# wusize/CLIPSelf

Hardware: AMD Instinct MI355X
Metric: images/sec (student+teacher distill step), ViT-B/16 32 crops/img (higher is better)
Workload: dtype bf16; 1 GPU; EVA02-CLIP-B-16 CLIPSelf image-patches step, 64 images x 32 crops per GPU, 224^2 (BASELINE configs[1]); global_batch=64, crops_per_image=32, image_size=224, parallelism=dp1, teacher_chunk=2048, teacher_last_block=cls_query_only, teacher_schedule=one_batch_ahead_on_side_stream

## Files before the change

### clipself_amd/csrc/gemm_stream.hip

```cpp
#include <vector>
#include <cstdio>
#include "gemm_common.h"

namespace {

typedef __attribute__((ext_vector_type(2))) unsigned u32x2;
typedef __attribute__((ext_vector_type(4))) unsigned u32x4;

constexpr unsigned OOB = 0xfffffff0u;

__device__ __forceinline__ float lane_bcast(int src_lane_x4, float v) {
    return __int_as_float(__builtin_amdgcn_ds_bpermute(src_lane_x4, __float_as_int(v)));
}
__device__ __forceinline__ unsigned pack2(float a, float b) {
    union { bf16x2 v; unsigned u; } pk;
    pk.v[0] = f2bf(a);
    pk.v[1] = f2bf(b);
    return pk.u;
}
__device__ __forceinline__ void swap32(unsigned& x, unsigned& y) {
    const u32x2 r = __builtin_amdgcn_permlane32_swap(x, y, false, false);
    x = r[0];
    y = r[1];
}
// ... 356 lines not shown

template <bool LN, bool AUX, int CP>
__device__ __forceinline__ void epi_swiglu_slab(const GemmArgs& p, const f32x16 (&acc)[4][2], int lane, int row0, int tn, int wn, const EpiOps& eo,
                                                char* slab) {
    const int l31 = lane & 31, hf = lane >> 5;
    const int hbase = tn * 128 + wn * 32;
    const bool colok = hbase < p.group;
    float nm[4], rs[4];
#pragma unroll
    for (int i = 0; i < 4; ++i) {
        rs[i] = LN ? eo.rstd[i] : 1.f;
        nm[i] = LN ? -eo.rstd[i] * eo.mean[i] : 0.f;
    }
    float ssum[4] = {0.f, 0.f, 0.f, 0.f}, ssq[4] = {0.f, 0.f, 0.f, 0.f};
    const int sl0 = hf << 4;
#pragma unroll
    for (int q = 0; q < 4; ++q) {
        float hv[4][4];
#pragma unroll
        for (int r = 0; r < 4; ++r) {
            const int e = q * 4 + r;
            const int sl = sl0 + ((8 * q + r) << 2);
            const float b1 = lane_bcast(sl, eo.cb), b2 = lane_bcast(sl + 128, eo.cb);
            float c1 = 0.f, c2 = 0.f;
            if (LN) { c1 = lane_bcast(sl, eo.cc); c2 = lane_bcast(sl + 128, eo.cc); }
#pragma unroll
            for (int i = 0; i < 4; ++i) {
                float u = acc[i][0][e], v = acc[i][1][e];
                if (LN) {
                    u = fmaf(rs[i], u, fmaf(nm[i], c1, b1));
                    v = fmaf(rs[i], v, fmaf(nm[i], c2, b2));
                } else {
                    u += b1;
                    v += b2;
                }
                hv[i][r] = silu_mul(u, v);
            }
        }
#pragma unroll
        for (int i = 0; i < 4; ++i) {
            const unsigned d0 = pack2(hv[i][0], hv[i][1]), d1 = pack2(hv[i][2], hv[i][3]);
            if (AUX) {
                ssum[i] = dot2_bf16(d1, 0x3f803f80u, dot2_bf16(d0, 0x3f803f80u, ssum[i]));
                ssq[i] = dot2_bf16(d1, d1, dot2_bf16(d0, d0, ssq[i]));
            }
            const int lrow = i * 32 + l31;
            const int s8 = (2 * q + hf) ^ (((lrow >> 1) & 3) << 1);
            *(uint2*)(slab + lrow * 64 + s8 * 8) = make_uint2(d0, d1);
        }
    }
    const __amdgpu_buffer_rsrc_t rc = make_rsrc((const __bf16*)p.C + (size_t)row0 * p.ldc + hbase);
    const int piece = lane & 3;
#pragma unroll
    for (int k = 0; k < 8; ++k) {
        const int lrow = (lane >> 2) + 16 * k;
        const uint4 w = *(const uint4*)(slab + lrow * 64 + ((piece ^ ((lrow >> 1) & 3)) << 4));
        const bool ok = colok && row0 + lrow < p.M && !CS_ABL(p, 8);
        store16<CP>(u32x4{w.x, w.y, w.z, w.w}, rc, ok ? (unsigned)(lrow * p.ldc + piece * 8) * 2u : OOB);
    }
    if (AUX) {
        const size_t slice = (size_t)tn * 4 + wn;
        const __amdgpu_buffer_rsrc_t rst = make_rsrc(p.stats_part + (slice * p.M + row0) * 2);
#pragma unroll
        for (int i = 0; i < 4; ++i) {
            const float s = both_halves(ssum[i]), q2 = both_halves(ssq[i]);
            const bool ok = colok && hf == 0 && row0 + i * 32 + l31 < p.M && !CS_ABL(p, 8);
            store8<CP>(u32x2{__float_as_uint(s), __float_as_uint(q2)}, rst, ok ? (unsigned)(i * 32 + l31) * 8u : OOB);
        }
    }
}

#ifdef CS_ABLATION_SWITCHES
__device__ unsigned long long* g_epi_trace = nullptr;
#define EPI_TRACE(slot)                                                                                                            \
    do {                                                                                                                           \
        if (g_epi_trace && (threadIdx.x & 63) == 0)                                                                                \
            g_epi_trace[((size_t)blockIdx.x * 8 + (threadIdx.x >> 6)) * 16 + (slot)] = __builtin_amdgcn_s_memrealtime();           \
    } while (0)
#define EPI_TRACE_WAIT() do { if (g_epi_trace) asm volatile("s_waitcnt vmcnt(0)" ::: "memory"); } while (0)
#else
#define EPI_TRACE(slot) do { } while (0)
#define EPI_TRACE_WAIT() do { } while (0)
#endif
template <bool LN, bool AUX, int CP, bool F8 = false, int SPLIT = 0, int FM = 4>
__device__ __forceinline__ void epi_resid_slab(const GemmArgs& p, const f32x16 (&acc)[FM][2], int lane, int row0, int colw, int tn, int wn,
                                               const EpiOps& eo, char* slab) {
    static_assert(!(SPLIT & 2) || AUX, "a split stream leaves together with the row statistics");
    const int l31 = lane & 31, hf = lane >> 5;
    const int rrow = lane >> 3, piece = lane & 7, col = colw + piece * 8;
    const bool colok = col < p.N;
    const __amdgpu_buffer_rsrc_t rc = make_rsrc((SPLIT & 2) ? (const void*)p.xb_out : (const void*)((const float*)p.C + (size_t)row0 * p.ldc + colw));
    const __amdgpu_buffer_rsrc_t rx = make_rsrc((SPLIT & 1) ? (const void*)p.xb_out : (const void*)(p.extra + (size_t)row0 * p.ldc + colw));
    const __amdgpu_buffer_rsrc_t rb = make_rsrc((AUX || SPLIT) ? (const void*)(p.xb_out + (size_t)row0 * p.ldxb + colw) : (const void*)p.C);
    const __amdgpu_buffer_rsrc_t rl = make_rsrc(SPLIT ? (const void*)(p.lo + (size_t)row0 * p.ldxb + colw) : (const void*)p.A);
    const size_t slice = (size_t)tn * 4 + wn;
    const __amdgpu_buffer_rsrc_t rst = make_rsrc(AUX ? (const void*)(p.stats_part + (slice * p.M + row0) * 2) : (const void*)p.C);
    f32x4 cb4[2] = {{0.f, 0.f, 0.f, 0.f}, {0.f, 0.f, 0.f, 0.f}}, cc4[2] = {{0.f, 0.f, 0.f, 0.f}, {0.f, 0.f, 0.f, 0.f}};
#pragma unroll
    for (int h = 0; h < 2; ++h) {
        const unsigned off = colok ? (unsigned)(col + 4 * h) * 4u : OOB;
        if (p.bias) cb4[h] = __builtin_bit_cast(f32x4, __builtin_amdgcn_raw_buffer_load_b128(make_rsrc(p.bias), off, 0, 0));
        if (LN || F8) cc4[h] = __builtin_bit_cast(f32x4, __builtin_amdgcn_raw_buffer_load_b128(make_rsrc(p.ln_colsum), off, 0, 0));
    }
    EPI_TRACE(0);
#pragma unroll
    for (int i = 0; i < FM; ++i) {
        f32x4 xin[4][2];
#pragma unroll
        for (int it = 0; it < 4; ++it) {
            const int rrel = i * 32 + rrow + 8 * it;
            const bool ok = colok && row0 + rrel < p.M;
            if constexpr (SPLIT & 1) {
                const unsigned off = ok ? (unsigned)(rrel * p.ldxb + piece * 8) * 2u : OOB;
                const u32x4 h = __builtin_bit_cast(u32x4, __builtin_amdgcn_raw_buffer_load_b128(rb, off, 0, CP));
                const u32x4 l = __builtin_bit_cast(u32x4, __builtin_amdgcn_raw_buffer_load_b128(rl, off, 0, CP));
#pragma unroll
                for (int w = 0; w < 4; ++w) {
                    xin[it][w >> 1][2 * (w & 1)] = __uint_as_float(__builtin_amdgcn_perm(h[w], l[w], 0x05040100u) - 0x8000u);
                    xin[it][w >> 1][2 * (w & 1) + 1] = __uint_as_float(__builtin_amdgcn_perm(h[w], l[w], 0x07060302u) - 0x8000u);
                }
            } else {
                const unsigned off = ok ? (unsigned)(rrel * p.ldc + piece * 8) * 4u : OOB;
                xin[it][0] = __builtin_bit_cast(f32x4, __builtin_amdgcn_raw_buffer_load_b128(rx, off, 0, CP));
                xin[it][1] = __builtin_bit_cast(f32x4, __builtin_amdgcn_raw_buffer_load_b128(rx, ok ? off + 16u : OOB, 0, CP));
            }
        }
        const float rs_row = (LN || F8) ? eo.rstd[i] : 1.f, nm_row = LN ? -eo.rstd[i] * eo.mean[i] : 0.f;
#pragma unroll
        for (int j = 0; j < 2; ++j)
#pragma unroll
            for (int q = 0; q < 4; ++q) {
                f32x4 t;
#pragma unroll
                for (int r = 0; r < 4; ++r) t[r] = acc[i][j][q * 4 + r];
                const int s16 = (j * 8 + 2 * q + hf) ^ (l31 & 15);
                *(f32x4*)(slab + l31 * 256 + s16 * 16) = t;
            }
        EPI_TRACE(1 + 3 * i);
        EPI_TRACE_WAIT();
        EPI_TRACE(2 + 3 * i);
        const int sel = lane & 7;
        float st_s = 0.f, st_q = 0.f;
#pragma unroll
        for (int it = 0; it < 4; ++it) {
            const int lrow = rrow + 8 * it, rrel = i * 32 + lrow;
            const bool ok = colok && row0 + rrel < p.M;
            float rs = 1.f, nm = 0.f;
            if (LN || F8) rs = lane_bcast(lrow << 2, rs_row);
            if (LN) nm = lane_bcast(lrow << 2, nm_row);
            f32x4 o[2];
#pragma unroll
            for (int h = 0; h < 2; ++h) {
                const f32x4 sv = *(const f32x4*)(slab + lrow * 256 + (((2 * piece + h) ^ (lrow & 15)) << 4));
                if (LN) {
#pragma unroll
                    for (int t = 0; t < 4; ++t) o[h][t] = xin[it][h][t] + fmaf(rs, sv[t], fmaf(nm, cc4[h][t], cb4[h][t]));
                } else if (F8) {
#pragma unroll
                    for (int t = 0; t < 4; ++t) o[h][t] = xin[it][h][t] + fmaf(rs * cc4[h][t], sv[t], cb4[h][t]);
                } else {
                    o[h] = xin[it][h] + (sv + cb4[h]);
                }
            }
            if constexpr (SPLIT & 2) {
                const unsigned off = ok ? (unsigned)(rrel * p.ldxb + piece * 8) * 2u : OOB;
                unsigned y[8];
#pragma unroll
                for (int t = 0; t < 8; ++t) y[t] = __float_as_uint(o[t >> 2][t & 3]) + 0x8000u;
                store16<CP>(u32x4{__builtin_amdgcn_perm(y[1], y[0], 0x07060302u), __builtin_amdgcn_perm(y[3], y[2], 0x07060302u),
                                  __builtin_amdgcn_perm(y[5], y[4], 0x07060302u), __builtin_amdgcn_perm(y[7], y[6], 0x07060302u)}, rb, off);
                store16<CP>(u32x4{__builtin_amdgcn_perm(y[1], y[0], 0x05040100u), __builtin_amdgcn_perm(y[3], y[2], 0x05040100u),
                                  __builtin_amdgcn_perm(y[5], y[4], 0x05040100u), __builtin_amdgcn_perm(y[7], y[6], 0x05040100u)}, rl, off);
            } else {
                const unsigned off = ok ? (unsigned)(rrel * p.ldc + piece * 8) * 4u : OOB;
                store16<CP>(__builtin_bit_cast(u32x4, o[0]), rc, off);
                store16<CP>(__builtin_bit_cast(u32x4, o[1]), rc, ok ? off + 16u : OOB);
            }
            if (AUX) {
                if constexpr (!(SPLIT & 2))
                    store16<CP>(u32x4{pack2(o[0][0], o[0][1]), pack2(o[0][2], o[0][3]), pack2(o[1][0], o[1][1]), pack2(o[1][2], o[1][3])}, rb,
                                ok ? (unsigned)(rrel * p.ldxb + piece * 8) * 2u : OOB);
                float ps = 0.f, pq = 0.f;
                if (colok) {
#pragma unroll
                    for (int t = 0; t < 8; ++t) { ps += o[t >> 2][t & 3]; pq = fmaf(o[t >> 2][t & 3], o[t >> 2][t & 3], pq); }
                }
                const float a = sum_lanes8(ps), b = sum_lanes8(pq);
                if (sel == it) { st_s = a; st_q = b; }
            }
        }
        if (AUX) {
            const int rrel = i * 32 + rrow + 8 * sel;
            const bool ok = sel < 4 && row0 + rrel < p.M && colw < p.N;
            store8<CP>(u32x2{__float_as_uint(st_s), __float_as_uint(st_q)}, rst, ok ? (unsigned)rrel * 8u : OOB);
        }
        EPI_TRACE(3 + 3 * i);
        __builtin_amdgcn_sched_barrier(0);
    }
}

template <int EPI, bool AUX, bool SLAB, int SPLIT = 0, int FM = 4, int MF = 32>
constexpr int epi_stores() {
    if (EPI == EPI_SWIGLU_BF16 && MF == 16) return 8 + (AUX ? 2 : 0);
    if (EPI == EPI_SWIGLU_BF16) return FM * (2 + (AUX ? 1 : 0));
    if (EPI == EPI_RESID_F32) return FM * (8 + (AUX ? ((SPLIT & 2) ? 0 : 4) + 1 : 0));
    return FM * 4;
}

#ifndef CS_DMA_AUX_A
#define CS_DMA_AUX_A 0
#endif
#ifndef CS_DMA_AUX_B
#define CS_DMA_AUX_B 0
#endif
#define CS_VMCNT(N) asm volatile("s_waitcnt vmcnt(%0)" ::"n"(N) : "memory")

inline bool getenv_flag(const char* name) {
    const char* v = getenv(name);
    return v && v[0] && v[0] != '0';
}

template <int EPI, bool LN, bool AUX, bool SLAB, bool F8 = false, int SPLIT = 0, int BMT = 256, int MF = 32>
__global__ __launch_bounds__(512) void gemm_stream_kernel(GemmArgs p) {
    static_assert(MF == 32 || (MF == 16 && LN && !SLAB && !F8 && SPLIT == 0 && BMT == 256 && (epi_is_bf16(EPI) ? !AUX : EPI == EPI_SWIGLU_BF16)),
                  "16x16x32 loop: the folded-LN bf16 and SwiGLU register epilogues");
    constexpr bool M16 = MF == 16;
    static_assert(BMT == 256 || (BMT == 192 && !F8 && SPLIT == 0 && !LN && !AUX), "192-row tiles: the training schedule's plain epilogues");
    static_assert(SPLIT == 0 || (EPI == EPI_RESID_F32 && LN && !F8), "the split stream belongs to the folded-LayerNorm residual epilogue");
    static_assert(SLAB || EPI != EPI_RESID_F32, "the fp32 residual epilogue exists in the slab form only (whole-line traffic)");
    static_assert(!F8 || (!LN && !AUX && (EPI == EPI_BF16 || EPI == EPI_RESID_F32)), "fp8 operands: bf16 and fp32-residual outputs");
    constexpr int ES = F8 ? 1 : 2;
    constexpr int CP = 0;
    constexpr bool SWI = EPI == EPI_SWIGLU_BF16, RES = EPI == EPI_RESID_F32;
    static_assert(SWI || RES || epi_is_bf16(EPI), "register epilogues");
    constexpr int BM = BMT, BN = 256, WN = 4, TM = BM / 2, TN = 64, FM = TM / 32, FN = 2;
    constexpr int A_BYTES = BM * BK * 2, B_BYTES = BN * BK * 2;
    constexpr int NPA = BM / 32;
    constexpr int NM = FM * FN, NR = FM + FN;
    constexpr int S = epi_stores<EPI, AUX, SLAB, SPLIT, FM, MF>() < 55 ? epi_stores<EPI, AUX, SLAB, SPLIT, FM, MF>() : 55;
    extern __shared__ __attribute__((aligned(16))) char smem[];
    const int tid = threadIdx.x, lane = tid & 63;
    const int wave = __builtin_amdgcn_readfirstlane(tid >> 6);
    const int wm = wave / WN, wn = wave - wm * WN;
    const int hf = M16 ? lane >> 4 : lane >> 5, l31 = M16 ? lane & 15 : lane & 31;
    char* const b_ring = smem + 3 * A_BYTES;
    const int ntiles = p.tiles_m * p.tiles_n, ktiles = p.K / (F8 ? 128 : BK);
    const int a_base = ((wm * TM + l31) >> 1) << 8, b_base = ((wn * TN + l31) >> 1) << 8;
    const int par8 = (l31 & 1) << 3, sw = l31 >> 1;
    const int G = gridDim.x;
#ifndef CS_NO_DMA_ROLES
    constexpr bool ROLES = !F8;
#else
    constexpr bool ROLES = false;
#endif
    const bool role_a = ROLES && wave >= 4;
#ifndef CS_NO_MID_BARRIER
    constexpr bool MID = ROLES && !SLAB && !F8;
#else
    constexpr bool MID = false;
#endif

    unsigned avoff[ROLES ? 8 : 4], bvoff[ROLES ? 1 : 4];
    const char *a_src = nullptr, *b_src = nullptr;
    int a_tile = blockIdx.x, a_kt = 0, b_tile = blockIdx.x, b_kt = 0;
    auto set_a = [&](int tile) {
        int tm, tn;
        tile_of_id(p, tile, ntiles, tm, tn);
        a_src = (const char*)p.A + (size_t)tm * BM * p.lda * ES;
#pragma unroll
        for (int i = 0; i < (ROLES ? NPA : 4); ++i) {
            int tr, chk;
            lane_source(ROLES ? (wave & 3) * NPA + i : wave * 4 + i, lane, tr, chk);
            avoff[i] = (unsigned)(min(tr, p.M - 1 - tm * BM) * p.lda * ES + chk * 16);
        }
    };
    auto set_b = [&](int tile) {
        int tm, tn;
        tile_of_id(p, tile, ntiles, tm, tn);
        if (SWI) {
            b_src = (const char*)p.B + (size_t)tn * (BN / 2) * p.ldb * ES;
        } else {
            b_src = (const char*)p.B + (size_t)tn * BN * p.ldb * ES;
        }
#pragma unroll
        for (int i = 0; i < (ROLES ? 8 : 4); ++i) {
            int tr, chk;
            lane_source(ROLES ? (wave & 3) * 8 + i : wave * 4 + i, lane, tr, chk);
            int rel;
            if (SWI) {
                const int hrel = (tr >> 6) * 32 + (tr & 31);
                rel = ((tr >> 5) & 1) * p.group + min(hrel, p.group - 1 - tn * (BN / 2));
            } else {
                rel = min(tr, p.N - 1 - tn * BN);
            }
            (ROLES ? avoff : bvoff)[i] = (unsigned)(rel * p.ldb * ES + chk * 16);
        }
    };
    auto adv_a = [&]() {
        if (++a_kt == ktiles) {
            a_kt = 0;
            if (a_tile + G < ntiles) {
                a_tile += G;
                set_a(a_tile);
            }
        }
    };
    auto adv_b = [&]() {
        if (++b_kt == ktiles) {
            b_kt = 0;
            if (b_tile + G < ntiles) {
                b_tile += G;
                set_b(b_tile);
            }
        }
    };
#define ISSUE_A(X, SLOT)                                                                                                      \
    __builtin_amdgcn_global_load_lds((const __attribute__((address_space(1))) void*)(a_src + (size_t)a_kt * (BK * 2) + avoff[X]), \
                                     (__attribute__((address_space(3))) void*)(smem + (SLOT) * A_BYTES + (wave * 4 + (X)) * 1024), 16, 0, CS_DMA_AUX_A)
#define ISSUE_B(X, SLOT)                                                                                                      \
    __builtin_amdgcn_global_load_lds((const __attribute__((address_space(1))) void*)(b_src + (size_t)b_kt * (BK * 2) + bvoff[X]), \
                                     (__attribute__((address_space(3))) void*)(b_ring + (SLOT) * B_BYTES + (wave * 4 + (X)) * 1024), 16, 0, CS_DMA_AUX_B)

#define ISSUE_RA(X, SLOT)                                                                                                     \
    __builtin_amdgcn_global_load_lds((const __attribute__((address_space(1))) void*)(a_src + (size_t)a_kt * (BK * 2) + avoff[X]), \
                                     (__attribute__((address_space(3))) void*)(smem + (SLOT) * A_BYTES + ((wave & 3) * NPA + (X)) * 1024), 16, 0, CS_DMA_AUX_A)
#define ISSUE_RB(X, SLOT)                                                                                                     \
    __builtin_amdgcn_global_load_lds((const __attribute__((address_space(1))) void*)(b_src + (size_t)b_kt * (BK * 2) + avoff[X]), \
                                     (__attribute__((address_space(3))) void*)(b_ring + (SLOT) * B_BYTES + ((wave & 3) * 8 + (X)) * 1024), 16, 0, CS_DMA_AUX_B)

    if constexpr (ROLES) {
        if (role_a) {
            set_a(a_tile);
#pragma unroll
            for (int x = 0; x < NPA; ++x) ISSUE_RA(x, 0);
            adv_a();
#pragma unroll
            for (int x = 0; x < NPA; ++x) ISSUE_RA(x, 1);
            adv_a();
        } else {
            set_b(b_tile);
#pragma unroll
            for (int x = 0; x < 8; ++x) ISSUE_RB(x, 0);
            adv_b();
            if constexpr (MID) {
#pragma unroll
                for (int x = 0; x < 8; ++x) ISSUE_RB(x, 1);
                adv_b();
            }
        }
        if constexpr (MID) {
            if (role_a) CS_VMCNT(NPA);
            else CS_VMCNT(8);
            __builtin_amdgcn_s_barrier();
        }
    } else {
        set_a(a_tile);
        set_b(b_tile);
#pragma unroll
        for (int x = 0; x < 4; ++x) ISSUE_A(x, 0);
        adv_a();
#pragma unroll
        for (int x = 0; x < 4; ++x) ISSUE_B(x, 0);
        adv_b();
#pragma unroll
        for (int x = 0; x < 4; ++x) ISSUE_A(x, 1);
        adv_a();
    }

    int curA = 0, gpar = 0;
    bool after_epi = false;
    for (int tile = blockIdx.x; tile < ntiles; tile += G) {
        int tm, tn;
        tile_of_id(p, tile, ntiles, tm, tn);
        const int row0 = tm * BM + wm * TM, colw = tn * BN + wn * TN;
        f32x16 acc[M16 ? 1 : FM][M16 ? 1 : FN];
        f32x4 acc16[M16 ? 8 : 1][M16 ? 4 : 1];
        constexpr int RB = M16 ? 16 : 32, NRB = TM / RB;
        EpiOpsT<M16 ? 8 : 4> eo;
        auto load_epi_ops = [&](int ln) {
            const int l31 = ln & (RB - 1), hf = ln >> 5, lane = ln;
#pragma unroll
            for (int i = 0; i < (M16 ? 8 : 4); ++i) eo.mean[i] = eo.rstd[i] = 0.f;
            eo.cb = eo.cc = 0.f;
            if (LN || F8) {
#pragma unroll
                for (int i = 0; i < NRB; ++i) {
                    const int r = min(row0 + i * RB + l31, p.M - 1);
                    if (LN) eo.mean[i] = p.ln_mean[r];
                    eo.rstd[i] = p.ln_rstd[r];
                }
            }
            int co;
            if (SWI) co = hf * p.group + min(tn * 128 + wn * 32 + (lane & 31), p.group - 1);
            else co = min(colw + lane, p.N - 1);
            if (!RES) {
                if (p.bias) eo.cb = p.bias[co];
                if (LN || F8) eo.cc = p.ln_colsum[co];
            }
        };

        auto ktile = [&](auto zero_tag, auto role_tag) {
            constexpr bool ZERO = decltype(zero_tag)::value;
            constexpr int ROLE = decltype(role_tag)::value;
            constexpr int KEEP = ROLE == 0 ? 4 : ROLE == 1 ? 0 : NPA;
            constexpr int SS = S + KEEP > 63 ? 63 - KEEP : S;
            if (after_epi) CS_VMCNT(KEEP + SS);
            else CS_VMCNT(KEEP);
            after_epi = false;
            asm volatile("s_waitcnt lgkmcnt(0)" ::: "memory");
            if (!CS_ABL(p, 2))
                __builtin_amdgcn_s_barrier();
            const char* la = smem + curA * A_BYTES + a_base;
            const char* lb = b_ring + gpar * B_BYTES + b_base;
            const int slot_a2 = curA == 0 ? 2 : curA - 1, slot_b1 = gpar ^ 1;
            if constexpr (F8) {
                typedef __attribute__((ext_vector_type(8))) int i32x8;
                typedef __attribute__((ext_vector_type(4))) int i32x4;
#pragma unroll
                for (int s2 = 0; s2 < 2; ++s2) {
                    const int c0 = 4 * s2 + 2 * hf;
                    const int off0 = ((par8 | c0) ^ sw) << 4, off1 = ((par8 | (c0 + 1)) ^ sw) << 4;
                    i32x8 a8[FM], b8[FN];
#pragma unroll
                    for (int i = 0; i < FM; ++i) {
                        const i32x4 lo = *(const i32x4*)(la + i * (16 * 256) + off0), hi = *(const i32x4*)(la + i * (16 * 256) + off1);
                        a8[i] = i32x8{lo[0], lo[1], lo[2], lo[3], hi[0], hi[1], hi[2], hi[3]};
                    }
#pragma unroll
                    for (int j = 0; j < FN; ++j) {
                        const i32x4 lo = *(const i32x4*)(lb + j * (16 * 256) + off0), hi = *(const i32x4*)(lb + j * (16 * 256) + off1);
                        b8[j] = i32x8{lo[0], lo[1], lo[2], lo[3], hi[0], hi[1], hi[2], hi[3]};
                    }
                    if constexpr (ROLE == 1) {
                        if (s2 == 0) {
#pragma unroll
                            for (int x = 0; x < 8; ++x) ISSUE_RB(x, slot_b1);
                        }
                    } else if constexpr (ROLE == 2) {
                        if (s2 == 1) {
#pragma unroll
                            for (int x = 0; x < NPA; ++x) ISSUE_RA(x, slot_a2);
                        }
                    } else if (s2 == 0) {
                        ISSUE_B(0, slot_b1); ISSUE_B(1, slot_b1); ISSUE_B(2, slot_b1); ISSUE_B(3, slot_b1);
                    } else {
                        ISSUE_A(0, slot_a2); ISSUE_A(1, slot_a2); ISSUE_A(2, slot_a2); ISSUE_A(3, slot_a2);
                    }
#pragma unroll
                    for (int i = 0; i < FM; ++i)
#pragma unroll
                        for (int j = 0; j < FN; ++j) {
                            if (ZERO && s2 == 0) {
                                const f32x16 z = {0.f, 0.f, 0.f, 0.f, 0.f, 0.f, 0.f, 0.f, 0.f, 0.f, 0.f, 0.f, 0.f, 0.f, 0.f, 0.f};
                                acc[i][j] = __builtin_amdgcn_mfma_scale_f32_32x32x64_f8f6f4(b8[j], a8[i], z, 0, 0, 0, 0x7f7f7f7f, 0, 0x7f7f7f7f);
                            } else {
                                acc[i][j] = __builtin_amdgcn_mfma_scale_f32_32x32x64_f8f6f4(b8[j], a8[i], acc[i][j], 0, 0, 0, 0x7f7f7f7f, 0, 0x7f7f7f7f);
                            }
                        }
                }
            } else {
                bf16x8 a[2][FM], b[2][FN];
                auto frags = [&](int ks, int buf) {
                    const int off = ((par8 | (ks * 2 + hf)) ^ sw) << 4;
#pragma unroll
                    for (int i = 0; i < FM; ++i) a[buf][i] = *(const bf16x8*)(la + i * (16 * 256) + off);
#pragma unroll
                    for (int j = 0; j < FN; ++j) b[buf][j] = *(const bf16x8*)(lb + j * (16 * 256) + off);
                };
                frags(0, 0);
#ifndef CS_NO_SGB
                __builtin_amdgcn_sched_group_barrier(0x100, 6, 0);
#endif
#pragma unroll
                for (int ks = 0; ks < 4; ++ks) {
                    const int cb = ks & 1;
                    if (ks < 3) frags(ks + 1, cb ^ 1);
                    if constexpr (ROLE == 1) {
                        if (ks == 0) { ISSUE_RB(0, slot_b1); ISSUE_RB(1, slot_b1); ISSUE_RB(2, slot_b1); ISSUE_RB(3, slot_b1); }
                        if (ks == 1) { ISSUE_RB(4, slot_b1); ISSUE_RB(5, slot_b1); ISSUE_RB(6, slot_b1); ISSUE_RB(7, slot_b1); }
                    } else if constexpr (ROLE == 2) {
                        if (ks == 2) {
#pragma unroll
                            for (int x = 0; x < NPA / 2; ++x) ISSUE_RA(x, slot_a2);
                        }
                        if (ks == 3) {
#pragma unroll
                            for (int x = NPA / 2; x < NPA; ++x) ISSUE_RA(x, slot_a2);
                        }
                    } else if (ks < 2) {
                        if ((ks & 1) == 0) { ISSUE_B(0, slot_b1); ISSUE_B(1, slot_b1); } else { ISSUE_B(2, slot_b1); ISSUE_B(3, slot_b1); }
                    } else {
                        if ((ks & 1) == 0) { ISSUE_A(0, slot_a2); ISSUE_A(1, slot_a2); } else { ISSUE_A(2, slot_a2); ISSUE_A(3, slot_a2); }
                    }
#pragma unroll
                    for (int i = 0; i < FM; ++i)
#pragma unroll
                        for (int j = 0; j < FN; ++j) {
                            if (ZERO && ks == 0) {
                                const f32x16 z = {0.f, 0.f, 0.f, 0.f, 0.f, 0.f, 0.f, 0.f, 0.f, 0.f, 0.f, 0.f, 0.f, 0.f, 0.f, 0.f};
                                acc[i][j] = __builtin_amdgcn_mfma_f32_32x32x16_bf16(b[cb][j], a[cb][i], z, 0, 0, 0);
                            } else {
                                acc[i][j] = __builtin_amdgcn_mfma_f32_32x32x16_bf16(b[cb][j], a[cb][i], acc[i][j], 0, 0, 0);
                            }
                        }
#ifndef CS_NO_SGB
                    const bool DMA4 = (ROLE == 1 && ks < 2) || (ROLE == 2 && ks >= 2);
                    constexpr int DN = ROLE == 2 ? NPA / 2 : 4;
#pragma unroll
                    for (int m = 0; m < NM; ++m) {
                        __builtin_amdgcn_sched_group_barrier(0x008, 1, 0);
                        if (ROLE == 0) {
                            if (m < NR) {
                                if (ks < 3) __builtin_amdgcn_sched_group_barrier(0x100, 1, 0);
                            } else {
                                __builtin_amdgcn_sched_group_barrier(0x010, 1, 0);
                            }
                        } else {
                            if (m < NR && ks < 3) __builtin_amdgcn_sched_group_barrier(0x100, 1, 0);
                            if (DMA4 && ks < 3 && m == NM - 2) __builtin_amdgcn_sched_group_barrier(0x010, 2, 0);
                            if (DMA4 && ks < 3 && m == NM - 1) __builtin_amdgcn_sched_group_barrier(0x010, DN - 2, 0);
                            if (DMA4 && ks == 3 && m >= 2 && m < 2 + DN) __builtin_amdgcn_sched_group_barrier(0x010, 1, 0);
                        }
                    }
#endif
                }
            }
            if (ROLE != 2) adv_b();
            if (ROLE != 1) adv_a();
            curA = curA == 2 ? 0 : curA + 1;
            gpar ^= 1;
        };
        bf16x8 fa[2][MID ? FM : 1], fb[2][MID ? FN : 1];
        auto ktile_mid = [&](auto zero_tag, auto role_tag) {
            constexpr bool ZERO = decltype(zero_tag)::value;
            constexpr int ROLE = decltype(role_tag)::value;
            const int nextA = curA == 2 ? 0 : curA + 1;
            const char* la = smem + curA * A_BYTES + a_base;
            const char* lb = b_ring + gpar * B_BYTES + b_base;
            const char* la_n = smem + nextA * A_BYTES + a_base;
            const char* lb_n = b_ring + (gpar ^ 1) * B_BYTES + b_base;
            const int slot_a2 = curA == 0 ? 2 : curA - 1, slot_b2 = gpar;
            auto frags = [&](const char* pa, const char* pb, int ks, int buf) {
                const int off = ((par8 | (ks * 2 + hf)) ^ sw) << 4;
#pragma unroll
                for (int i = 0; i < FM; ++i) fa[buf][i] = *(const bf16x8*)(pa + i * (16 * 256) + off);
#pragma unroll
                for (int j = 0; j < FN; ++j) fb[buf][j] = *(const bf16x8*)(pb + j * (16 * 256) + off);
            };
            auto mfmas = [&](int cb, bool zero) {
#pragma unroll
                for (int i = 0; i < FM; ++i)
#pragma unroll
                    for (int j = 0; j < FN; ++j) {
                        if (zero) {
                            const f32x16 z = {0.f, 0.f, 0.f, 0.f, 0.f, 0.f, 0.f, 0.f, 0.f, 0.f, 0.f, 0.f, 0.f, 0.f, 0.f, 0.f};
                            acc[i][j] = __builtin_amdgcn_mfma_f32_32x32x16_bf16(fb[cb][j], fa[cb][i], z, 0, 0, 0);
                        } else {
                            acc[i][j] = __builtin_amdgcn_mfma_f32_32x32x16_bf16(fb[cb][j], fa[cb][i], acc[i][j], 0, 0, 0);
                        }
                    }
            };
            if (ZERO) {
                frags(la, lb, 0, 0);
                __builtin_amdgcn_sched_group_barrier(0x100, 6, 0);
            }
#pragma unroll
            for (int ks = 0; ks < 3; ++ks) {
                const int cb = ks & 1;
                frags(la, lb, ks + 1, cb ^ 1);
                constexpr int KA = 1;
                if constexpr (ROLE == 2) {
                    if (ks == KA) {
#pragma unroll
                        for (int x = 0; x < NPA / 2; ++x) ISSUE_RA(x, slot_a2);
                    }
                    if (ks == KA + 1) {
#pragma unroll
                        for (int x = NPA / 2; x < NPA; ++x) ISSUE_RA(x, slot_a2);
                    }
                }
                mfmas(cb, ZERO && ks == 0);
#pragma unroll
                for (int m = 0; m < NM; ++m) {
                    __builtin_amdgcn_sched_group_barrier(0x008, 1, 0);
                    if (m < NR) __builtin_amdgcn_sched_group_barrier(0x100, 1, 0);
                    if (ROLE == 2 && (ks == KA || ks == KA + 1) && m == NM - 2) __builtin_amdgcn_sched_group_barrier(0x010, 2, 0);
                    if (ROLE == 2 && (ks == KA || ks == KA + 1) && m == NM - 1) __builtin_amdgcn_sched_group_barrier(0x010, NPA / 2 - 2, 0);
                }
            }
            {
                constexpr int KEEP = ROLE == 1 ? 0 : NPA;
                constexpr int SS = S + KEEP > 63 ? 63 - KEEP : S;
                if (after_epi) CS_VMCNT(KEEP + SS);
                else CS_VMCNT(KEEP);
                after_epi = false;
                asm volatile("s_waitcnt lgkmcnt(0)" ::: "memory");
                __builtin_amdgcn_s_barrier();
            }
            {
                const int off = ((par8 | hf) ^ sw) << 4;
#pragma unroll
                for (int x = 0; x < 8; ++x) {
                    if (x < FM) fa[0][x] = *(const bf16x8*)(la_n + x * (16 * 256) + off);
                    else if (x < NR) fb[0][x - FM] = *(const bf16x8*)(lb_n + (x - FM) * (16 * 256) + off);
                    if constexpr (ROLE == 1) ISSUE_RB(x, slot_b2);
                }
            }
            mfmas(1, false);
#pragma unroll
            for (int m = 0; m < NM; ++m) {
                __builtin_amdgcn_sched_group_barrier(0x008, 1, 0);
                if (m < NR) __builtin_amdgcn_sched_group_barrier(0x100, 1, 0);
                if (ROLE == 1 && m < NM - 1) __builtin_amdgcn_sched_group_barrier(0x010, 1, 0);
                if (ROLE == 1 && m == NM - 1) __builtin_amdgcn_sched_group_barrier(0x010, 1 + 8 - NM, 0);
            }
            if (ROLE == 1) adv_b();
            else adv_a();
            curA = nextA;
            gpar ^= 1;
        };
        bf16x8 ga[2][M16 ? 4 : 1], gb[M16 ? 4 : 1];
        auto ktile_m16 = [&](auto zero_tag, auto role_tag) {
            constexpr bool ZERO = decltype(zero_tag)::value;
            constexpr int ROLE = decltype(role_tag)::value;
            const int nextA = curA == 2 ? 0 : curA + 1;
            const char* la = smem + curA * A_BYTES + a_base;
            const char* lb = b_ring + gpar * B_BYTES + b_base;
            const char* la_n = smem + nextA * A_BYTES + a_base;
            const char* lb_n = b_ring + (gpar ^ 1) * B_BYTES + b_base;
            const int slot_a2 = curA == 0 ? 2 : curA - 1, slot_b2 = gpar;
            auto frag = [&](const char* base, int ks, int blk) {
                const int off = (((par8 | (ks * 4 + hf)) ^ sw) << 4) ^ ((blk & 1) << 7);
                return *(const bf16x8*)(base + blk * (8 * 256) + off);
            };
            auto read_a = [&](const char* pa, int ks, int c) {
#pragma unroll
                for (int x = 0; x < 4; ++x) ga[c][x] = frag(pa, ks, c * 4 + x);
            };
            auto read_b = [&](const char* pb, int ks, int jj) {
                gb[2 * jj] = frag(pb, ks, 2 * jj);
                gb[2 * jj + 1] = frag(pb, ks, 2 * jj + 1);
            };
            auto mfmas = [&](int c, int jj, bool zero) {
#pragma unroll
                for (int x = 0; x < 4; ++x)
#pragma unroll
                    for (int j = 2 * jj; j < 2 * jj + 2; ++j) {
                        if (zero) {
                            const f32x4 z = {0.f, 0.f, 0.f, 0.f};
                            acc16[c * 4 + x][j] = __builtin_amdgcn_mfma_f32_16x16x32_bf16(gb[j], ga[c][x], z, 0, 0, 0);
                        } else {
                            acc16[c * 4 + x][j] = __builtin_amdgcn_mfma_f32_16x16x32_bf16(gb[j], ga[c][x], acc16[c * 4 + x][j], 0, 0, 0);
                        }
                    }
            };
            auto order = [&](auto r0a, auto nra, auto r0b, auto nrb, auto d0a, auto nda, auto d0b, auto ndb) {
#pragma unroll
                for (int m = 0; m < 16; ++m) {
                    __builtin_amdgcn_sched_group_barrier(0x008, 1, 0);
                    if ((m >= r0a.value && m < r0a.value + nra.value) || (m >= r0b.value && m < r0b.value + nrb.value))
                        __builtin_amdgcn_sched_group_barrier(0x100, 1, 0);
                    if ((m >= d0a.value && m < d0a.value + nda.value) || (m >= d0b.value && m < d0b.value + ndb.value))
                        __builtin_amdgcn_sched_group_barrier(0x010, 1, 0);
                }
            };
#define CI(N) std::integral_constant<int, (N)>{}
            if (ZERO) {
                read_a(la, 0, 0);
                read_b(lb, 0, 0);
                __builtin_amdgcn_sched_group_barrier(0x100, 6, 0);
            }
            read_b(lb, 0, 1);
            mfmas(0, 0, ZERO);
            read_a(la, 0, 1);
            mfmas(0, 1, ZERO);
            order(CI(0), CI(2), CI(8), CI(4), CI(0), CI(0), CI(0), CI(0));
            read_a(la, 1, 0);
            mfmas(1, 0, ZERO);
            read_b(lb, 1, 0);
            if constexpr (ROLE == 2) {
#pragma unroll
                for (int x = 0; x < NPA / 2; ++x) ISSUE_RA(x, slot_a2);
            }
            mfmas(1, 1, ZERO);
            order(CI(0), CI(4), CI(8), CI(2), CI(10), CI(ROLE == 2 ? NPA / 2 : 0), CI(0), CI(0));
            read_b(lb, 1, 1);
            if constexpr (ROLE == 2) {
#pragma unroll
                for (int x = NPA / 2; x < NPA; ++x) ISSUE_RA(x, slot_a2);
            }
            mfmas(0, 0, false);
            read_a(la, 1, 1);
            mfmas(0, 1, false);
            order(CI(0), CI(2), CI(8), CI(4), CI(2), CI(ROLE == 2 ? NPA / 2 : 0), CI(0), CI(0));
            {
                constexpr int KEEP = ROLE == 1 ? 0 : NPA;
                constexpr int SS = S + KEEP > 63 ? 63 - KEEP : S;
                if (after_epi) CS_VMCNT(KEEP + SS);
                else CS_VMCNT(KEEP);
                after_epi = false;
                asm volatile("s_waitcnt lgkmcnt(0)" ::: "memory");
                __builtin_amdgcn_s_barrier();
            }
            read_a(la_n, 0, 0);
            if constexpr (ROLE == 1) { ISSUE_RB(0, slot_b2); ISSUE_RB(1, slot_b2); ISSUE_RB(2, slot_b2); ISSUE_RB(3, slot_b2); }
            mfmas(1, 0, false);
            read_b(lb_n, 0, 0);
            if constexpr (ROLE == 1) { ISSUE_RB(4, slot_b2); ISSUE_RB(5, slot_b2); ISSUE_RB(6, slot_b2); ISSUE_RB(7, slot_b2); }
            mfmas(1, 1, false);
            order(CI(0), CI(4), CI(8), CI(2), CI(4), CI(ROLE == 1 ? 4 : 0), CI(10), CI(ROLE == 1 ? 4 : 0));
#undef CI
            if (ROLE == 1) adv_b();
            else adv_a();
            curA = nextA;
            gpar ^= 1;
        };
        if constexpr (M16) {
            if (role_a) {
                ktile_m16(std::true_type{}, std::integral_constant<int, 2>{});
                for (int kt = 1; kt < ktiles; ++kt) ktile_m16(std::false_type{}, std::integral_constant<int, 2>{});
            } else {
                ktile_m16(std::true_type{}, std::integral_constant<int, 1>{});
                for (int kt = 1; kt < ktiles; ++kt) ktile_m16(std::false_type{}, std::integral_constant<int, 1>{});
            }
        } else if constexpr (MID) {
            if (role_a) {
                ktile_mid(std::true_type{}, std::integral_constant<int, 2>{});
                for (int kt = 1; kt < ktiles; ++kt) ktile_mid(std::false_type{}, std::integral_constant<int, 2>{});
            } else {
                ktile_mid(std::true_type{}, std::integral_constant<int, 1>{});
                for (int kt = 1; kt < ktiles; ++kt) ktile_mid(std::false_type{}, std::integral_constant<int, 1>{});
            }
        } else if constexpr (ROLES) {
            if (role_a) {
                ktile(std::true_type{}, std::integral_constant<int, 2>{});
                for (int kt = 1; kt < ktiles; ++kt) ktile(std::false_type{}, std::integral_constant<int, 2>{});
            } else {
                ktile(std::true_type{}, std::integral_constant<int, 1>{});
                for (int kt = 1; kt < ktiles; ++kt) ktile(std::false_type{}, std::integral_constant<int, 1>{});
            }
        } else {
            ktile(std::true_type{}, std::integral_constant<int, 0>{});
            for (int kt = 1; kt < ktiles; ++kt) ktile(std::false_type{}, std::integral_constant<int, 0>{});
        }
        if (CS_ABL(p, 4)) continue;
        after_epi = true;
        int lane_e = lane;
        asm volatile("" : "+v"(lane_e));
        if constexpr (SLAB) {
            asm volatile("s_waitcnt lgkmcnt(0)" ::: "memory");
            __builtin_amdgcn_s_barrier();
            char* const slab = wave >= 4 ? b_ring + (gpar ^ 1) * B_BYTES + (wave - 4) * 8192
                               : (BM == 192 && wave == 3) ? b_ring + 2 * B_BYTES
                                                          : smem + (curA == 0 ? 2 : curA - 1) * A_BYTES + wave * 8192;
            load_epi_ops(lane_e);
#ifndef CS_NO_KERNARG_RELOAD
            constexpr bool RELOAD = RES && LN && AUX;
#else
            constexpr bool RELOAD = false;
#endif
            if constexpr (RELOAD) {
                const __attribute__((address_space(4))) GemmArgs* pk = (const __attribute__((address_space(4))) GemmArgs*)__builtin_amdgcn_kernarg_segment_ptr();
                asm volatile("" : "+s"(pk));
                GemmArgs pe;
                pe.A = pk->A; pe.C = pk->C; pe.bias = pk->bias; pe.extra = pk->extra; pe.M = pk->M; pe.N = pk->N; pe.ldc = pk->ldc;
                pe.ln_colsum = pk->ln_colsum; pe.stats_part = pk->stats_part; pe.xb_out = pk->xb_out; pe.ldxb = pk->ldxb; pe.lo = pk->lo;
                pe.dbg = pk->dbg;
                epi_resid_slab<LN, AUX, CP, F8, SPLIT, FM>(pe, acc, lane_e, row0, colw, tn, wn, eo, slab);
            } else if constexpr (RES) {
                epi_resid_slab<LN, AUX, CP, F8, SPLIT, FM>(p, acc, lane_e, row0, colw, tn, wn, eo, slab);
            } else {
                static_assert(FM == 4, "the slab forms of the bf16 / SwiGLU epilogues exist for 256-row tiles");
                if constexpr (SWI) epi_swiglu_slab<LN, AUX, CP>(p, acc, lane_e, row0, tn, wn, eo, slab);
                else epi_bf16_slab<epi_act(EPI), LN, CP>(p, acc, lane_e, row0, colw, eo, slab);
            }
        } else {
            load_epi_ops(lane_e);
            if constexpr (M16 && SWI) epi_swiglu_m16<LN, AUX, CP>(p, acc16, lane_e, row0, tn, wn, eo);
            else if constexpr (M16) epi_bf16_m16<epi_act(EPI), LN, CP>(p, acc16, lane_e, row0, colw, eo);
            else if constexpr (SWI) epi_swiglu<LN, AUX, CP, FM>(p, acc, lane_e, row0, tn, wn, eo);
            else epi_bf16<epi_act(EPI), LN, CP, F8, FM>(p, acc, lane_e, row0, colw, eo);
        }
    }
    CS_VMCNT(0);
#undef ISSUE_A
#undef ISSUE_B
#undef ISSUE_RA
#undef ISSUE_RB
}

template <int EPI, bool LN, bool AUX, bool SLAB, int BMT = 256, int MF = 32>
int launch_stream_v(const GemmArgs& a, unsigned grid, hipStream_t stream) {
    constexpr size_t lds = 160 * 1024;
    static bool once = ((void)hipFuncSetAttribute((const void*)gemm_stream_kernel<EPI, LN, AUX, SLAB, false, 0, BMT, MF>, hipFuncAttributeMaxDynamicSharedMemorySize, (int)lds), true);
    (void)once;
    hipLaunchKernelGGL((gemm_stream_kernel<EPI, LN, AUX, SLAB, false, 0, BMT, MF>), dim3(grid), dim3(512), lds, stream, a);
    CS_LAUNCH_CHECK();
    return 0;
}

template <int EPI, bool LN, bool AUX>
int launch_stream_t(const GemmArgs& a, unsigned grid, hipStream_t stream) {
    if constexpr (EPI == EPI_RESID_F32) return launch_stream_v<EPI, LN, AUX, true>(a, grid, stream);
    else if (a.dbg & 1) return launch_stream_v<EPI, LN, AUX, true>(a, grid, stream);
    else if constexpr (LN && (epi_is_bf16(EPI) ? !AUX : EPI == EPI_SWIGLU_BF16)) {
        if (!getenv_flag("CS_GEMM_MFMA32")) return launch_stream_v<EPI, LN, AUX, false, 256, 16>(a, grid, stream);
        return launch_stream_v<EPI, LN, AUX, false>(a, grid, stream);
    } else return launch_stream_v<EPI, LN, AUX, false>(a, grid, stream);
}

template <bool AUX, int SPLIT>
int launch_stream_split(const GemmArgs& a, unsigned grid, hipStream_t stream) {
    constexpr size_t lds = 160 * 1024;
    static bool once = ((void)hipFuncSetAttribute((const void*)gemm_stream_kernel<EPI_RESID_F32, true, AUX, true, false, SPLIT>,
                                                  hipFuncAttributeMaxDynamicSharedMemorySize, (int)lds), true);
    (void)once;
    hipLaunchKernelGGL((gemm_stream_kernel<EPI_RESID_F32, true, AUX, true, false, SPLIT>), dim3(grid), dim3(512), lds, stream, a);
    CS_LAUNCH_CHECK();
    return 0;
}

template <int EPI>
int launch_stream_bf16(const GemmArgs& a, unsigned grid, hipStream_t stream) {
    return a.ln_mean ? launch_stream_t<EPI, true, false>(a, grid, stream) : launch_stream_t<EPI, false, false>(a, grid, stream);
}

template <int EPI, bool SLAB>
int launch_stream_f8(const GemmArgs& a, unsigned grid, hipStream_t stream) {
    constexpr size_t lds = 160 * 1024;
    static bool once = ((void)hipFuncSetAttribute((const void*)gemm_stream_kernel<EPI, false, false, SLAB, true>, hipFuncAttributeMaxDynamicSharedMemorySize, (int)lds), true);
    (void)once;
    hipLaunchKernelGGL((gemm_stream_kernel<EPI, false, false, SLAB, true>), dim3(grid), dim3(512), lds, stream, a);
    CS_LAUNCH_CHECK();
    return 0;
}

}

int cs_gemm_stream_launch_f8(GemmArgs a, int epi, int reserve, hipStream_t stream) {
    a.tiles_m = (a.M + 255) / 256;
    a.tiles_n = (a.N + 255) / 256;
    const long ntiles = (long)a.tiles_m * a.tiles_n;
    const long cap = cs_persistent_cap(reserve);
    const unsigned grid = (unsigned)(ntiles < cap ? ntiles : cap);
    if (epi == EPI_BF16) return launch_stream_f8<EPI_BF16, false>(a, grid, stream);
    return launch_stream_f8<EPI_RESID_F32, true>(a, grid, stream);
}

#ifdef CS_ABLATION_SWITCHES
static int stream_launch_impl(GemmArgs a, int epi, int reserve, hipStream_t stream);
int cs_gemm_stream_launch(GemmArgs a, int epi, int reserve, hipStream_t stream) {
    static const char* path = getenv("CS_GEMM_TRACE");
    static unsigned long long* buf = nullptr;
    constexpr size_t WORDS = 256 * 8 * 16;
    if (path && !buf && hipMalloc((void**)&buf, WORDS * 8) == hipSuccess) {
        (void)hipMemset(buf, 0, WORDS * 8);
        (void)hipMemcpyToSymbol(HIP_SYMBOL(g_epi_trace), &buf, sizeof(buf));
    }
    const int rc = stream_launch_impl(a, epi, reserve, stream);
    if (path && buf && rc == 0 && (epi == EPI_RESID_F32 || epi == EPI_RESID_LN_F32)) {
        (void)hipStreamSynchronize(stream);
        std::vector<unsigned long long> host(WORDS);
        (void)hipMemcpy(host.data(), buf, WORDS * 8, hipMemcpyDeviceToHost);
        if (FILE* f = fopen(path, "wb")) { fwrite(host.data(), 8, WORDS, f); fclose(f); }
    }
    return rc;
}
static int stream_launch_impl(GemmArgs a, int epi, int reserve, hipStream_t stream) {
#else
int cs_gemm_stream_launch(GemmArgs a, int epi, int reserve, hipStream_t stream) {
#endif
    const bool swi = epi == EPI_SWIGLU_BF16, res = epi == EPI_RESID_F32 || epi == EPI_RESID_LN_F32;
    if (!(swi || res || epi == EPI_BF16 || epi == EPI_QGELU_BF16)) return 1;
    if (a.M < 1 || a.K % BK != 0) return 1;
    if (swi ? (a.group % 32 != 0) : (a.N % 32 != 0)) return 1;
    if ((long)a.ldc * 128 * 4 >= 0x70000000L || (long)a.ldxb * 128 * 2 >= 0x70000000L) return 1;
    const bool ln = a.ln_mean != nullptr;
    if ((epi == EPI_RESID_LN_F32) != (res && ln)) return 1;
    bool aux = false;
    if (swi) aux = a.stats_part != nullptr;
    else if (res) {
        if ((a.stats_part != nullptr) != (a.xb_out != nullptr)) return 1;
        aux = a.stats_part != nullptr;
        if (aux && (a.ldxb % 8 != 0 || ((uintptr_t)a.xb_out % 16) != 0)) return 1;
    } else if (a.stats_part || a.xb_out) return 1;
    a.tiles_m = (a.M + 255) / 256;
    a.tiles_n = swi ? (a.group + 127) / 128 : (a.N + 255) / 256;
    long ntiles = (long)a.tiles_m * a.tiles_n;
    const long cap = cs_persistent_cap(reserve);
    unsigned grid = (unsigned)(ntiles < cap ? ntiles : cap);
    if (!ln && !aux && !(a.dbg & 1) && a.M >= 192 && (swi || res || epi == EPI_BF16) && !getenv_flag("CS_NO_BM192")) {
        const long t192 = (long)((a.M + 191) / 192) * a.tiles_n;
        const long c256 = ((ntiles + cap - 1) / cap) * 256, c192 = ((t192 + cap - 1) / cap) * 192;
        if (c192 * 10 < c256 * 9) {
            a.tiles_m = (a.M + 191) / 192;
            ntiles = t192;
            grid = (unsigned)(ntiles < cap ? ntiles : cap);
            if (swi) return launch_stream_v<EPI_SWIGLU_BF16, false, false, false, 192>(a, grid, stream);
            if (res) return launch_stream_v<EPI_RESID_F32, false, false, true, 192>(a, grid, stream);
            return launch_stream_v<EPI_BF16, false, false, false, 192>(a, grid, stream);
        }
    }
// ... 67 lines not shown
```

Measured before the change: 764.3 images/sec.

## Use 16x16x32 MFMA K-loop for folded-LN residual slab GEMMs with large K

Extends the 16x16x32 bf16 MFMA main loop to the fp32 residual slab-epilogue kernels, including the split-stream variants. It adds a scheduled K-tile with interleaved LDS reads, MFMAs and DMA issues, plus a 16x16 accumulator layout path in the slab epilogue. The path is selected by default when K >= 2048, which covers the MLP down-projection, and can be overridden by environment variables. The change risks higher register pressure and recomputing lane-dependent offsets per tile, since it forces an opaque lane copy and redoes set_a/set_b every tile.

```diff
diff --git a/clipself_amd/csrc/gemm_stream.hip b/clipself_amd/csrc/gemm_stream.hip
--- a/clipself_amd/csrc/gemm_stream.hip
+++ b/clipself_amd/csrc/gemm_stream.hip
@@ -462,10 +462,11 @@
 #define EPI_TRACE(slot) do { } while (0)
 #define EPI_TRACE_WAIT() do { } while (0)
 #endif
-template <bool LN, bool AUX, int CP, bool F8 = false, int SPLIT = 0, int FM = 4>
-__device__ __forceinline__ void epi_resid_slab(const GemmArgs& p, const f32x16 (&acc)[FM][2], int lane, int row0, int colw, int tn, int wn,
-                                               const EpiOps& eo, char* slab) {
+template <bool LN, bool AUX, int CP, bool F8 = false, int SPLIT = 0, int FM = 4, int MF = 32, typename ACC, typename EO>
+__device__ __forceinline__ void epi_resid_slab(const GemmArgs& p, const ACC& acc, int lane, int row0, int colw, int tn, int wn,
+                                               const EO& eo, char* slab) {
     static_assert(!(SPLIT & 2) || AUX, "a split stream leaves together with the row statistics");
+    static_assert(MF == 32 || (MF == 16 && FM == 4 && !F8), "16x16 accumulators: 256-row tiles of the bf16 kernels");
     const int l31 = lane & 31, hf = lane >> 5;
     const int rrow = lane >> 3, piece = lane & 7, col = colw + piece * 8;
     const bool colok = col < p.N;
@@ -506,16 +507,27 @@
             }
         }
         const float rs_row = (LN || F8) ? eo.rstd[i] : 1.f, nm_row = LN ? -eo.rstd[i] * eo.mean[i] : 0.f;
-#pragma unroll
-        for (int j = 0; j < 2; ++j)
-#pragma unroll
-            for (int q = 0; q < 4; ++q) {
-                f32x4 t;
-#pragma unroll
-                for (int r = 0; r < 4; ++r) t[r] = acc[i][j][q * 4 + r];
-                const int s16 = (j * 8 + 2 * q + hf) ^ (l31 & 15);
-                *(f32x4*)(slab + l31 * 256 + s16 * 16) = t;
-            }
+        if constexpr (MF == 16) {
+            const int l15 = lane & 15, g = lane >> 4;
+#pragma unroll
+            for (int b = 0; b < 2; ++b)
+#pragma unroll
+                for (int j = 0; j < 4; ++j) {
+                    const int s16 = (4 * j + g) ^ l15;
+                    *(f32x4*)(slab + (b * 16 + l15) * 256 + s16 * 16) = acc[2 * i + b][j];
+                }
+        } else {
+#pragma unroll
+            for (int j = 0; j < 2; ++j)
+#pragma unroll
+                for (int q = 0; q < 4; ++q) {
+                    f32x4 t;
+#pragma unroll
+                    for (int r = 0; r < 4; ++r) t[r] = acc[i][j][q * 4 + r];
+                    const int s16 = (j * 8 + 2 * q + hf) ^ (l31 & 15);
+                    *(f32x4*)(slab + l31 * 256 + s16 * 16) = t;
+                }
+        }
         EPI_TRACE(1 + 3 * i);
         EPI_TRACE_WAIT();
         EPI_TRACE(2 + 3 * i);
@@ -602,8 +614,9 @@
 
 template <int EPI, bool LN, bool AUX, bool SLAB, bool F8 = false, int SPLIT = 0, int BMT = 256, int MF = 32>
 __global__ __launch_bounds__(512) void gemm_stream_kernel(GemmArgs p) {
-    static_assert(MF == 32 || (MF == 16 && LN && !SLAB && !F8 && SPLIT == 0 && BMT == 256 && (epi_is_bf16(EPI) ? !AUX : EPI == EPI_SWIGLU_BF16)),
-                  "16x16x32 loop: the folded-LN bf16 and SwiGLU register epilogues");
+    static_assert(MF == 32 || (MF == 16 && LN && !F8 && BMT == 256 &&
+                                (EPI == EPI_RESID_F32 ? SLAB : !SLAB && SPLIT == 0 && (epi_is_bf16(EPI) ? !AUX : EPI == EPI_SWIGLU_BF16))),
+                  "16x16x32 loop: the folded-LN bf16 and SwiGLU register epilogues, the folded-LN residual slab epilogue");
     constexpr bool M16 = MF == 16;
     static_assert(BMT == 256 || (BMT == 192 && !F8 && SPLIT == 0 && !LN && !AUX), "192-row tiles: the training schedule's plain epilogues");
     static_assert(SPLIT == 0 || (EPI == EPI_RESID_F32 && LN && !F8), "the split stream belongs to the folded-LayerNorm residual epilogue");
@@ -642,6 +655,7 @@
 
     unsigned avoff[ROLES ? 8 : 4], bvoff[ROLES ? 1 : 4];
     const char *a_src = nullptr, *b_src = nullptr;
+    int lane_d = lane;
     int a_tile = blockIdx.x, a_kt = 0, b_tile = blockIdx.x, b_kt = 0;
     auto set_a = [&](int tile) {
         int tm, tn;
@@ -650,7 +664,7 @@
 #pragma unroll
         for (int i = 0; i < (ROLES ? NPA : 4); ++i) {
             int tr, chk;
-            lane_source(ROLES ? (wave & 3) * NPA + i : wave * 4 + i, lane, tr, chk);
+            lane_source(ROLES ? (wave & 3) * NPA + i : wave * 4 + i, lane_d, tr, chk);
             avoff[i] = (unsigned)(min(tr, p.M - 1 - tm * BM) * p.lda * ES + chk * 16);
         }
     };
@@ -665,7 +679,7 @@
 #pragma unroll
         for (int i = 0; i < (ROLES ? 8 : 4); ++i) {
             int tr, chk;
-            lane_source(ROLES ? (wave & 3) * 8 + i : wave * 4 + i, lane, tr, chk);
+            lane_source(ROLES ? (wave & 3) * 8 + i : wave * 4 + i, lane_d, tr, chk);
             int rel;
             if (SWI) {
                 const int hrel = (tr >> 6) * 32 + (tr & 31);
@@ -753,14 +767,24 @@
         int tm, tn;
         tile_of_id(p, tile, ntiles, tm, tn);
         const int row0 = tm * BM + wm * TM, colw = tn * BN + wn * TN;
+        int lane_k = lane;
+        if constexpr (M16 && SLAB) {
+            asm volatile("" : "+v"(lane_k));
+            lane_d = lane_k;
+            if (role_a) set_a(a_tile);
+            else set_b(b_tile);
+        }
+        const int hf_k = lane_k >> 4, l15_k = lane_k & 15;
+        const int a_base_k = ((wm * TM + l15_k) >> 1) << 8, b_base_k = ((wn * TN + l15_k) >> 1) << 8;
+        const int par8_k = (l15_k & 1) << 3, sw_k = l15_k >> 1;
         f32x16 acc[M16 ? 1 : FM][M16 ? 1 : FN];
         f32x4 acc16[M16 ? 8 : 1][M16 ? 4 : 1];
-        constexpr int RB = M16 ? 16 : 32, NRB = TM / RB;
-        EpiOpsT<M16 ? 8 : 4> eo;
+        constexpr int RB = M16 && !RES ? 16 : 32, NRB = TM / RB;
+        EpiOpsT<RB == 16 ? 8 : 4> eo;
         auto load_epi_ops = [&](int ln) {
             const int l31 = ln & (RB - 1), hf = ln >> 5, lane = ln;
 #pragma unroll
-            for (int i = 0; i < (M16 ? 8 : 4); ++i) eo.mean[i] = eo.rstd[i] = 0.f;
+            for (int i = 0; i < (RB == 16 ? 8 : 4); ++i) eo.mean[i] = eo.rstd[i] = 0.f;
             eo.cb = eo.cc = 0.f;
             if (LN || F8) {
 #pragma unroll
@@ -838,6 +862,76 @@
                             }
                         }
                 }
+            } else if constexpr (M16) {
+                static_assert(ROLE != 0 && FM == 4, "the 16x16x32 K tile exists with DMA roles, for 256-row tiles");
+                bf16x8 ga[2][4], gb[4];
+                const char* la_k = smem + curA * A_BYTES + a_base_k;
+                const char* lb_k = b_ring + gpar * B_BYTES + b_base_k;
+                auto frag = [&](const char* base, int ks, int blk) {
+                    const int off = (((par8_k | (ks * 4 + hf_k)) ^ sw_k) << 4) ^ ((blk & 1) << 7);
+                    return *(const bf16x8*)(base + blk * (8 * 256) + off);
+                };
+                auto read_a = [&](int ks, int c) {
+#pragma unroll
+                    for (int x = 0; x < 4; ++x) ga[c][x] = frag(la_k, ks, c * 4 + x);
+                };
+                auto read_b = [&](int ks, int jj) {
+                    gb[2 * jj] = frag(lb_k, ks, 2 * jj);
+                    gb[2 * jj + 1] = frag(lb_k, ks, 2 * jj + 1);
+                };
+                auto mfmas = [&](int c, int jj, bool zero) {
+#pragma unroll
+                    for (int x = 0; x < 4; ++x)
+#pragma unroll
+                        for (int j = 2 * jj; j < 2 * jj + 2; ++j) {
+                            if (zero) {
+                                const f32x4 z = {0.f, 0.f, 0.f, 0.f};
+                                acc16[c * 4 + x][j] = __builtin_amdgcn_mfma_f32_16x16x32_bf16(gb[j], ga[c][x], z, 0, 0, 0);
+                            } else {
+                                acc16[c * 4 + x][j] = __builtin_amdgcn_mfma_f32_16x16x32_bf16(gb[j], ga[c][x], acc16[c * 4 + x][j], 0, 0, 0);
+                            }
+                        }
+                };
+                auto order = [&](auto r0a, auto nra, auto r0b, auto nrb, auto d0, auto nd) {
+#ifndef CS_NO_SGB
+#pragma unroll
+                    for (int m = 0; m < 16; ++m) {
+                        __builtin_amdgcn_sched_group_barrier(0x008, 1, 0);
+                        if ((m >= r0a.value && m < r0a.value + nra.value) || (m >= r0b.value && m < r0b.value + nrb.value))
+                            __builtin_amdgcn_sched_group_barrier(0x100, 1, 0);
+                        if (m >= d0.value && m < d0.value + nd.value) __builtin_amdgcn_sched_group_barrier(0x010, 1, 0);
+                    }
+#endif
+                };
+#define CI(N) std::integral_constant<int, (N)>{}
+                read_a(0, 0);
+                read_b(0, 0);
+#ifndef CS_NO_SGB
+                __builtin_amdgcn_sched_group_barrier(0x100, 6, 0);
+#endif
+                read_b(0, 1);
+                mfmas(0, 0, ZERO);
+                read_a(0, 1);
+                if constexpr (ROLE == 1) { ISSUE_RB(0, slot_b1); ISSUE_RB(1, slot_b1); ISSUE_RB(2, slot_b1); ISSUE_RB(3, slot_b1); }
+                mfmas(0, 1, ZERO);
+                order(CI(0), CI(2), CI(8), CI(4), CI(12), CI(ROLE == 1 ? 4 : 0));
+                read_a(1, 0);
+                mfmas(1, 0, ZERO);
+                read_b(1, 0);
+                if constexpr (ROLE == 1) { ISSUE_RB(4, slot_b1); ISSUE_RB(5, slot_b1); ISSUE_RB(6, slot_b1); ISSUE_RB(7, slot_b1); }
+                mfmas(1, 1, ZERO);
+                order(CI(0), CI(4), CI(8), CI(2), CI(10), CI(ROLE == 1 ? 4 : 0));
+                read_b(1, 1);
+                mfmas(0, 0, false);
+                read_a(1, 1);
+                if constexpr (ROLE == 2) { ISSUE_RA(0, slot_a2); ISSUE_RA(1, slot_a2); ISSUE_RA(2, slot_a2); ISSUE_RA(3, slot_a2); }
+                mfmas(0, 1, false);
+                order(CI(0), CI(2), CI(8), CI(4), CI(12), CI(ROLE == 2 ? 4 : 0));
+                if constexpr (ROLE == 2) { ISSUE_RA(4, slot_a2); ISSUE_RA(5, slot_a2); ISSUE_RA(6, slot_a2); ISSUE_RA(7, slot_a2); }
+                mfmas(1, 0, false);
+                mfmas(1, 1, false);
+                order(CI(0), CI(0), CI(0), CI(0), CI(2), CI(ROLE == 2 ? 4 : 0));
+#undef CI
             } else {
                 bf16x8 a[2][FM], b[2][FN];
                 auto frags = [&](int ks, int buf) {
@@ -999,7 +1093,7 @@
             curA = nextA;
             gpar ^= 1;
         };
-        bf16x8 ga[2][M16 ? 4 : 1], gb[M16 ? 4 : 1];
+        bf16x8 ga[2][M16 && !SLAB ? 4 : 1], gb[M16 && !SLAB ? 4 : 1];
         auto ktile_m16 = [&](auto zero_tag, auto role_tag) {
             constexpr bool ZERO = decltype(zero_tag)::value;
             constexpr int ROLE = decltype(role_tag)::value;
@@ -1095,7 +1189,7 @@
             curA = nextA;
             gpar ^= 1;
         };
-        if constexpr (M16) {
+        if constexpr (M16 && !SLAB) {
             if (role_a) {
                 ktile_m16(std::true_type{}, std::integral_constant<int, 2>{});
                 for (int kt = 1; kt < ktiles; ++kt) ktile_m16(std::false_type{}, std::integral_constant<int, 2>{});
@@ -1146,9 +1240,11 @@
                 pe.A = pk->A; pe.C = pk->C; pe.bias = pk->bias; pe.extra = pk->extra; pe.M = pk->M; pe.N = pk->N; pe.ldc = pk->ldc;
                 pe.ln_colsum = pk->ln_colsum; pe.stats_part = pk->stats_part; pe.xb_out = pk->xb_out; pe.ldxb = pk->ldxb; pe.lo = pk->lo;
                 pe.dbg = pk->dbg;
-                epi_resid_slab<LN, AUX, CP, F8, SPLIT, FM>(pe, acc, lane_e, row0, colw, tn, wn, eo, slab);
+                if constexpr (M16) epi_resid_slab<LN, AUX, CP, F8, SPLIT, FM, 16>(pe, acc16, lane_e, row0, colw, tn, wn, eo, slab);
+                else epi_resid_slab<LN, AUX, CP, F8, SPLIT, FM>(pe, acc, lane_e, row0, colw, tn, wn, eo, slab);
             } else if constexpr (RES) {
-                epi_resid_slab<LN, AUX, CP, F8, SPLIT, FM>(p, acc, lane_e, row0, colw, tn, wn, eo, slab);
+                if constexpr (M16) epi_resid_slab<LN, AUX, CP, F8, SPLIT, FM, 16>(p, acc16, lane_e, row0, colw, tn, wn, eo, slab);
+                else epi_resid_slab<LN, AUX, CP, F8, SPLIT, FM>(p, acc, lane_e, row0, colw, tn, wn, eo, slab);
             } else {
                 static_assert(FM == 4, "the slab forms of the bf16 / SwiGLU epilogues exist for 256-row tiles");
                 if constexpr (SWI) epi_swiglu_slab<LN, AUX, CP>(p, acc, lane_e, row0, tn, wn, eo, slab);
@@ -1167,6 +1263,11 @@
 #undef ISSUE_B
 #undef ISSUE_RA
 #undef ISSUE_RB
+}
+
+inline bool resid_mfma16(int K) {
+    if (getenv_flag("CS_GEMM_MFMA32")) return false;
+    return K >= 2048 || getenv_flag("CS_GEMM_RESID_MFMA16");
 }
 
 template <int EPI, bool LN, bool AUX, bool SLAB, int BMT = 256, int MF = 32>
@@ -1181,7 +1282,10 @@
 
 template <int EPI, bool LN, bool AUX>
 int launch_stream_t(const GemmArgs& a, unsigned grid, hipStream_t stream) {
-    if constexpr (EPI == EPI_RESID_F32) return launch_stream_v<EPI, LN, AUX, true>(a, grid, stream);
+    if constexpr (EPI == EPI_RESID_F32 && LN) {
+        if (resid_mfma16(a.K)) return launch_stream_v<EPI, LN, AUX, true, 256, 16>(a, grid, stream);
+        return launch_stream_v<EPI, LN, AUX, true>(a, grid, stream);
+    } else if constexpr (EPI == EPI_RESID_F32) return launch_stream_v<EPI, LN, AUX, true>(a, grid, stream);
     else if (a.dbg & 1) return launch_stream_v<EPI, LN, AUX, true>(a, grid, stream);
     else if constexpr (LN && (epi_is_bf16(EPI) ? !AUX : EPI == EPI_SWIGLU_BF16)) {
         if (!getenv_flag("CS_GEMM_MFMA32")) return launch_stream_v<EPI, LN, AUX, false, 256, 16>(a, grid, stream);
@@ -1189,15 +1293,20 @@
     } else return launch_stream_v<EPI, LN, AUX, false>(a, grid, stream);
 }
 
+template <bool AUX, int SPLIT, int MF>
+int launch_stream_split_v(const GemmArgs& a, unsigned grid, hipStream_t stream) {
+    constexpr size_t lds = 160 * 1024;
+    static bool once = ((void)hipFuncSetAttribute((const void*)gemm_stream_kernel<EPI_RESID_F32, true, AUX, true, false, SPLIT, 256, MF>,
+                                                  hipFuncAttributeMaxDynamicSharedMemorySize, (int)lds), true);
+    (void)once;
+    hipLaunchKernelGGL((gemm_stream_kernel<EPI_RESID_F32, true, AUX, true, false, SPLIT, 256, MF>), dim3(grid), dim3(512), lds, stream, a);
+    CS_LAUNCH_CHECK();
+    return 0;
+}
 template <bool AUX, int SPLIT>
 int launch_stream_split(const GemmArgs& a, unsigned grid, hipStream_t stream) {
-    constexpr size_t lds = 160 * 1024;
-    static bool once = ((void)hipFuncSetAttribute((const void*)gemm_stream_kernel<EPI_RESID_F32, true, AUX, true, false, SPLIT>,
-                                                  hipFuncAttributeMaxDynamicSharedMemorySize, (int)lds), true);
-    (void)once;
-    hipLaunchKernelGGL((gemm_stream_kernel<EPI_RESID_F32, true, AUX, true, false, SPLIT>), dim3(grid), dim3(512), lds, stream, a);
-    CS_LAUNCH_CHECK();
-    return 0;
+    if (resid_mfma16(a.K)) return launch_stream_split_v<AUX, SPLIT, 16>(a, grid, stream);
+    return launch_stream_split_v<AUX, SPLIT, 32>(a, grid, stream);
 }
 
 template <int EPI>
```

Result: no change. 768.3 images/sec, median of 6 (+0.5%).
